# TongtongSong/OpenEAT

Measured on AMD Instinct MI355X. Metric: audio-frames/sec/GPU (train) + RTF (attention-rescoring decode), 12L Conformer, higher is better.
Workload: dtype f32 (storage, accumulate, softmax, norms, losses, optimizer all fp32; every matrix product is the fp32 product to within one fp32 rounding, computed as six exact bf16 x bf16 MFMA products of three-piece operand splits h+m+l = x, dropped terms < 2^-24 |a||b| - tests hold it to the exact-fp32 mode's t; 1 GPU; configs[1]: 12L Conformer d=256 (12+3+3, h=4, ff=1024, K=15, V=3246), B=32/GPU x 10 s 16 kHz wav (T=998 frames), L=30, CTC+attention joint loss, fbank+fwd+bwd+clip+Adam, dropout 0.1; global_batch=32, parallelism=dp1, hip_graph=True

## Files before the change

### openeat_amd/csrc/gemm_tn.hip

```cpp
#include <stdlib.h>
#include "gemm_common.h"
#include "../../include/openeat_hip.h"

typedef __bf16 bf16x8 __attribute__((ext_vector_type(8)));
typedef __bf16 bf16x4 __attribute__((ext_vector_type(4)));
typedef short s16x4 __attribute__((ext_vector_type(4)));

#define TN_KROWS 32
#define TN_COLS 128
#define TN_PITCH (TN_COLS + 16)
#define TN_PLANE (TN_KROWS * TN_PITCH)
#define TN_THREADS 512

#ifdef OE_GEMM_STAMPS
static __device__ unsigned long long* tn_stamp_buf = nullptr;
extern "C" int oe_debug_set_tn_stamp_buffer(void* p) { return (int)hipMemcpyToSymbol(HIP_SYMBOL(tn_stamp_buf), &p, sizeof(p)); }
#define TN_NOW(var)                                                                          \
    do {                                                                                     \
        __builtin_amdgcn_sched_barrier(0);                                                   \
        asm volatile("s_memtime %0\n\ts_waitcnt lgkmcnt(0)" : "=s"(var) :: "memory");        \
        __builtin_amdgcn_sched_barrier(0);                                                   \
    } while (0)
#define TN_ACC(slot) do { unsigned long long t1_; TN_NOW(t1_); tn_acc[slot] += t1_ - tn_t; tn_t = t1_; } while (0)
#else
#define TN_NOW(var) do { } while (0)
#define TN_ACC(slot) do { } while (0)
#endif

template <int TERMS> struct TFrag { bf16x8 p[oe_npl<TERMS>::N]; };

template <int TERMS>
__device__ __forceinline__ void tn_frag(const __bf16* img, int col32, int s, int lane, TFrag<TERMS>& f) {
    const int i = lane & 15, grp = lane >> 4;
    const __bf16* p = img + (16 * s + 4 * (grp >> 1) + (i >> 2)) * TN_PITCH + col32 + 16 * (grp & 1) + 4 * (i & 3);
    typedef __attribute__((address_space(3))) s16x4 lds_s16x4;
#pragma unroll
    for (int n = 0; n < oe_npl<TERMS>::N; ++n) {
        union { s16x4 h[2]; bf16x8 v; } u;
        u.h[0] = __builtin_amdgcn_ds_read_tr16_b64_v4i16((lds_s16x4*)(p + n * TN_PLANE));
        u.h[1] = __builtin_amdgcn_ds_read_tr16_b64_v4i16((lds_s16x4*)(p + n * TN_PLANE + 8 * TN_PITCH));
        f.p[n] = u.v;
    }
}

template <int TERMS>
__device__ __forceinline__ f32x16 tn_mma(const TFrag<TERMS>& a, const TFrag<TERMS>& b, f32x16 c) {
    return oe_mma_terms<TERMS>(a, b, c);
}

struct TnRegs { float4 v[2]; };
__device__ __forceinline__ void tn_load(TnRegs& t, const float* base, long ld, int k0, int k_last) {
#pragma unroll
    for (int i = 0; i < 2; ++i) {
        const int k = min(k0 + (int)(threadIdx.x >> 5) + 16 * i, k_last);
        t.v[i] = *reinterpret_cast<const float4*>(base + (long)k * ld);
    }
}
template <int TERMS>
__device__ __forceinline__ void tn_store(const TnRegs& t, __bf16* img, int k0, int k_end) {
#pragma unroll
    for (int i = 0; i < 2; ++i) {
        const int row = (int)(threadIdx.x >> 5) + 16 * i;
        const bool live = k0 + row < k_end;
        const float x[4] = {live ? t.v[i].x : 0.f, live ? t.v[i].y : 0.f, live ? t.v[i].z : 0.f, live ? t.v[i].w : 0.f};
        constexpr int NPL = oe_npl<TERMS>::N;
        bf16x4 pl[NPL];
#pragma unroll
        for (int e = 0; e < 4; ++e) {
            __bf16 q[NPL];
            oe_split_bf16<NPL>(x[e], q);
#pragma unroll
            for (int n = 0; n < NPL; ++n) pl[n][e] = q[n];
        }
        __bf16* d = img + row * TN_PITCH + 4 * (threadIdx.x & 31);
#pragma unroll
        for (int n = 0; n < NPL; ++n) *reinterpret_cast<bf16x4*>(d + n * TN_PLANE) = pl[n];
    }
}

template <int TERMS>
__device__ __forceinline__ void tn_block(const float* __restrict__ Ap, long lda, const float* __restrict__ Bp, long ldb,
                                         float* __restrict__ C, long ldc, int M, int N, int Mr, int Nr, int K, int k_chunk,
                                         int tile_x, int tile_y, int tile_z, const EpiParams& ep) {
    constexpr int NPL = oe_npl<TERMS>::N;
    constexpr int OP_ELEMS = NPL * TN_PLANE;
    constexpr int BUF_ELEMS = 2 * OP_ELEMS;
    constexpr int XCH_BYTES = 4 * 2 * 32 * 64 * 4;
    constexpr int IMG_ELEMS = (2 * BUF_ELEMS * 2 >= XCH_BYTES) ? 2 * BUF_ELEMS : XCH_BYTES / 2;
    __shared__ __attribute__((aligned(16))) __bf16 img[IMG_ELEMS];
    __shared__ float csum_s[TN_COLS];

    const int lane = threadIdx.x & 63;
    const int wave = __builtin_amdgcn_readfirstlane(threadIdx.x >> 6);
    const int grp = wave >> 2, wm = (wave >> 1) & 1, wn = wave & 1;
    const long m0 = (long)tile_y * TN_COLS, n0 = (long)tile_x * TN_COLS;
    const int k_begin = tile_z * k_chunk;
    const int k_end = min(K, k_begin + k_chunk);
    const int nchunks = (k_end - k_begin + TN_KROWS - 1) / TN_KROWS;

    const int c4 = 4 * (threadIdx.x & 31);
    const float* a_src = Ap + min(m0 + c4, (long)Mr - 4);
    const float* b_src = Bp + min(n0 + c4, (long)Nr - 4);
    const bool do_csum = ep.a_colsum != nullptr && tile_x == 0;
    float cs[4] = {0.f, 0.f, 0.f, 0.f};

    f32x16 acc[2][2];
#pragma unroll
    for (int i = 0; i < 2; ++i)
#pragma unroll
        for (int j = 0; j < 2; ++j)
#pragma unroll
            for (int r = 0; r < 16; ++r) acc[i][j][r] = 0.f;

#ifdef OE_GEMM_STAMPS
    unsigned long long tn_acc[8] = {0, 0, 0, 0, 0, 0, 0, 0}, tn_t, tn_t0;
    TN_NOW(tn_t);
    tn_t0 = tn_t;
#endif
    TnRegs ra, rb;
    if (nchunks > 0) {
        tn_load(ra, a_src, lda, k_begin, k_end - 1);
        tn_load(rb, b_src, ldb, k_begin, k_end - 1);
        if (do_csum) {
#pragma unroll
            for (int i = 0; i < 2; ++i)
                if (k_begin + (int)(threadIdx.x >> 5) + 16 * i < k_end) { cs[0] += ra.v[i].x; cs[1] += ra.v[i].y; cs[2] += ra.v[i].z; cs[3] += ra.v[i].w; }
        }
        tn_store<TERMS>(ra, img, k_begin, k_end);
        tn_store<TERMS>(rb, img + OP_ELEMS, k_begin, k_end);
    }
    __syncthreads();
    TN_ACC(0);
    for (int c = 0; c < nchunks; ++c) {
        const int kn = k_begin + (c + 1) * TN_KROWS;
        const bool more = c + 1 < nchunks;
        if (more) {
            tn_load(ra, a_src, lda, kn, k_end - 1);
            tn_load(rb, b_src, ldb, kn, k_end - 1);
        }
        TN_ACC(1);
        const __bf16* ia = img + (c & 1) * BUF_ELEMS;
        const __bf16* ib = ia + OP_ELEMS;
        TFrag<TERMS> fa[2], fb[2];
        tn_frag<TERMS>(ia, wm * 64, grp, lane, fa[0]);
        tn_frag<TERMS>(ia, wm * 64 + 32, grp, lane, fa[1]);
        tn_frag<TERMS>(ib, wn * 64, grp, lane, fb[0]);
        tn_frag<TERMS>(ib, wn * 64 + 32, grp, lane, fb[1]);
#pragma unroll
        for (int i = 0; i < 2; ++i)
#pragma unroll
            for (int j = 0; j < 2; ++j) acc[i][j] = tn_mma<TERMS>(fa[i], fb[j], acc[i][j]);
        TN_ACC(2);
#ifdef OE_GEMM_STAMPS
        asm volatile("s_waitcnt vmcnt(0)" ::: "memory");
        TN_ACC(3);
#endif
        if (more) {
            if (do_csum) {
#pragma unroll
                for (int i = 0; i < 2; ++i)
                    if (kn + (int)(threadIdx.x >> 5) + 16 * i < k_end) { cs[0] += ra.v[i].x; cs[1] += ra.v[i].y; cs[2] += ra.v[i].z; cs[3] += ra.v[i].w; }
            }
            __bf16* nx = img + ((c + 1) & 1) * BUF_ELEMS;
            tn_store<TERMS>(ra, nx, kn, k_end);
            tn_store<TERMS>(rb, nx + OP_ELEMS, kn, k_end);
        }
        TN_ACC(4);
        __syncthreads();
        TN_ACC(5);
    }

    float alpha = ep.alpha;
    if (ep.alpha_dev) alpha *= *ep.alpha_dev;

    if (do_csum) {
        if (threadIdx.x < TN_COLS) csum_s[threadIdx.x] = 0.f;
        __syncthreads();
#pragma unroll
        for (int e = 0; e < 4; ++e) {
            const float v = cs[e] + __shfl_xor(cs[e], 32, 64);
            if (lane < 32) atomicAdd(&csum_s[4 * lane + e], v);
        }
        __syncthreads();
        if (threadIdx.x < TN_COLS && m0 + threadIdx.x < M) atomicAdd(ep.a_colsum + m0 + threadIdx.x, csum_s[threadIdx.x] * alpha);
    }

    float* xch = reinterpret_cast<float*>(img);
    const int q = wave & 3;
    {
        float* mine = xch + ((q * 2 + grp) * 32) * 64 + lane;
#pragma unroll
        for (int j = 0; j < 2; ++j)
#pragma unroll
            for (int r = 0; r < 16; ++r) mine[(j * 16 + r) * 64] = grp == 0 ? acc[1][j][r] : acc[0][j][r];
    }
    __syncthreads();
    f32x16 fin[2];
    {
        const float* theirs = xch + ((q * 2 + (1 - grp)) * 32) * 64 + lane;
#pragma unroll
        for (int j = 0; j < 2; ++j)
#pragma unroll
            for (int r = 0; r < 16; ++r) fin[j][r] = (grp == 0 ? acc[0][j][r] : acc[1][j][r]) + theirs[(j * 16 + r) * 64];
    }
    const int lrow = lane & 31, lk = lane >> 5;
    const bool interior = (m0 + TN_COLS <= M) && (n0 + TN_COLS <= N);
#pragma unroll
    for (int j = 0; j < 2; ++j) {
        const long col = n0 + wn * 64 + j * 32 + lrow;
        const long row0 = m0 + wm * 64 + grp * 32 + 4 * lk;
        float* base = C + row0 * ldc + col;
#pragma unroll
        for (int r = 0; r < 16; ++r) {
            const int dr = (r & 3) + 8 * (r >> 2);
            if (!interior && !(row0 + dr < M && col < N)) continue;
            const float v = fin[j][r] * alpha;
            if (ep.atomic) atomicAdd(base + dr * ldc, v);
            else if (ep.accumulate) base[dr * ldc] += v;
            else base[dr * ldc] = v;
        }
    }
#ifdef OE_GEMM_STAMPS
    TN_ACC(6);
    if (tn_stamp_buf && threadIdx.x == 0 && blockIdx.x < 2048) {
        for (int i = 0; i < 7; ++i) tn_stamp_buf[blockIdx.x * 8 + i] = tn_acc[i];
        tn_stamp_buf[blockIdx.x * 8 + 7] = tn_t - tn_t0;
    }
#endif
}

__device__ __forceinline__ int tn_swizzle(int id, int nblk) {
    const int q = nblk >> 3, r = nblk & 7, xcd = id & 7, j = id >> 3;
    return (xcd < r ? xcd * (q + 1) : r * (q + 1) + (xcd - r) * q) + j;
}

template <int TERMS>
__global__ __launch_bounds__(TN_THREADS) void gemm_tn_planes_kernel(const float* __restrict__ Ap, long lda, const float* __restrict__ Bp, long ldb,
                                                                   float* __restrict__ C, long ldc, int M, int N, int Mr, int Nr, int K, int k_chunk,
                                                                   int gx, int gy, EpiParams ep) {
    const int swz = tn_swizzle(blockIdx.x, gridDim.x);
    tn_block<TERMS>(Ap, lda, Bp, ldb, C, ldc, M, N, Mr, Nr, K, k_chunk, swz % gx, (swz / gx) % gy, swz / (gx * gy), ep);
}

template <int TERMS>
__global__ __launch_bounds__(TN_THREADS) void gemm_tn_grouped_kernel(const oe_tn_problem* __restrict__ tab, int n_problems) {
    const int swz = tn_swizzle(blockIdx.x, gridDim.x);
    int p = 0;
    while (p + 1 < n_problems && tab[p + 1].block_start <= swz) ++p;
    const oe_tn_problem pr = tab[p];
    const int local = swz - pr.block_start;
    EpiParams ep{};
    ep.alpha = pr.alpha; ep.alpha_dev = pr.alpha_dev; ep.beta = 1.f; ep.atomic = 1; ep.a_colsum = pr.a_colsum;
    tn_block<TERMS>(pr.a, pr.lda, pr.b, pr.ldb, pr.c, pr.ldc, pr.m, pr.n, (pr.m + 3) / 4 * 4, (pr.n + 3) / 4 * 4, pr.k, pr.k_chunk,
                    local % pr.gx, (local / pr.gx) % pr.gy, local / (pr.gx * pr.gy), ep);
}

extern "C" int oe_gemm_tn_grouped_plan(oe_tn_problem* problems, int n, int target_blocks) {
    OE_REQUIRE(problems && n > 0 && target_blocks > 0, "oe_gemm_tn_grouped_plan: bad arguments");
    long tiles = 0;
    for (int i = 0; i < n; ++i) {
        oe_tn_problem& p = problems[i];
        OE_REQUIRE(p.a && p.b && p.c && p.m >= 4 && p.n >= 4 && p.k >= 1, "oe_gemm_tn_grouped_plan: problem %d: bad shape / null pointer", i);
        OE_REQUIRE((((uintptr_t)p.a | (uintptr_t)p.b) & 15) == 0 && p.lda % 4 == 0 && p.ldb % 4 == 0 && p.lda >= (p.m + 3) / 4 * 4 &&
                       p.ldb >= (p.n + 3) / 4 * 4 && p.ldc >= p.n,
                   "oe_gemm_tn_grouped_plan: problem %d: operands not 16-byte aligned / leading dimensions too short", i);
        p.gx = oe_cdiv(p.n, TN_COLS);
        p.gy = oe_cdiv(p.m, TN_COLS);
        tiles += (long)p.gx * p.gy;
    }
    const int split = (int)min(16L, max(1L, (target_blocks + tiles / 2) / tiles));
    int blocks = 0;
    for (int i = 0; i < n; ++i) {
        oe_tn_problem& p = problems[i];
        int nz = min(split, max(1, p.k / 128));
        p.k_chunk = oe_cdiv(oe_cdiv(p.k, nz), TN_KROWS) * TN_KROWS;
        p.nz = oe_cdiv(p.k, p.k_chunk);
        p.block_start = blocks;
        blocks += p.gx * p.gy * p.nz;
    }
    return blocks;
}

extern "C" int oe_gemm_tn_grouped(const oe_tn_problem* problems_dev, int n, int total_blocks, int precision, void* stream) {
    OE_REQUIRE(problems_dev && n > 0 && total_blocks > 0, "oe_gemm_tn_grouped: bad arguments");
    OE_REQUIRE(precision == 1 || precision == 3 || precision == 6, "oe_gemm_tn_grouped: precision must be 1 (bf16), 3 (bf16x3) or 6 (bf16x6)");
    if (precision == 6)
        hipLaunchKernelGGL((gemm_tn_grouped_kernel<6>), dim3(total_blocks), dim3(TN_THREADS), 0, (hipStream_t)stream, problems_dev, n);
    else if (precision == 3)
        hipLaunchKernelGGL((gemm_tn_grouped_kernel<3>), dim3(total_blocks), dim3(TN_THREADS), 0, (hipStream_t)stream, problems_dev, n);
    else
        hipLaunchKernelGGL((gemm_tn_grouped_kernel<1>), dim3(total_blocks), dim3(TN_THREADS), 0, (hipStream_t)stream, problems_dev, n);
    OE_LAUNCH_CHECK("oe_gemm_tn_grouped");
    return 0;
}

int oe_gemm_tn_planes_try(const OperandDesc& A, const OperandDesc& B, float* C, long ldc, int M, int N, int K, int sk, const EpiParams& ep,
                          int terms, hipStream_t st) {
    static const int mode = getenv("OE_GEMM_TN_PLANES") ? atoi(getenv("OE_GEMM_TN_PLANES")) : 1;
    if (!mode) return 1;
    const int Mr = (M + 3) / 4 * 4, Nr = (N + 3) / 4 * 4;
    if (!A.vec_ok || !B.vec_ok || A.ld < Mr || B.ld < Nr || M < 4 || N < 4 || K < 1) return 1;
    if (ep.bias || ep.act || ep.preact_out || ep.actgrad_in || ep.residual || ep.rowmask || ep.drop_p > 0.f || ep.beta != 1.f || ep.scatter) return 1;
    if (sk > 1 && !ep.atomic) return 1;
    const int gx = oe_cdiv(N, TN_COLS), gy = oe_cdiv(M, TN_COLS);
    if (mode == 1 && (gx * gy < 12 || K < 2048)) return 1;
    int nz = 1;
    static const int blocks_target = getenv("OE_TN_BLOCKS") ? atoi(getenv("OE_TN_BLOCKS")) : 256;
    if (ep.atomic) {
        nz = max(1, blocks_target / (gx * gy));
        nz = min(nz, max(1, K / 128));
    }
    int kc = oe_cdiv(oe_cdiv(K, nz), TN_KROWS) * TN_KROWS;
    nz = oe_cdiv(K, kc);
    if (terms == 6)
        hipLaunchKernelGGL((gemm_tn_planes_kernel<6>), dim3(gx * gy * nz), dim3(TN_THREADS), 0, st, A.p, A.ld, B.p, B.ld, C, ldc, M, N, Mr, Nr, K, kc, gx, gy, ep);
    else if (terms == 3)
        hipLaunchKernelGGL((gemm_tn_planes_kernel<3>), dim3(gx * gy * nz), dim3(TN_THREADS), 0, st, A.p, A.ld, B.p, B.ld, C, ldc, M, N, Mr, Nr, K, kc, gx, gy, ep);
    else
        hipLaunchKernelGGL((gemm_tn_planes_kernel<1>), dim3(gx * gy * nz), dim3(TN_THREADS), 0, st, A.p, A.ld, B.p, B.ld, C, ldc, M, N, Mr, Nr, K, kc, gx, gy, ep);
    OE_LAUNCH_CHECK("oe_gemm (bf16 mfma, k-major planes)");
    return 0;
}
```

### openeat_amd/ops.py

```python
from __future__ import annotations

import itertools
import os
import math
import weakref
from typing import Optional

import torch

from . import hip
from . import arena as _arena
from . import planes as _planes

ACT_NONE, ACT_RELU, ACT_SWISH, ACT_TANH, ACT_HARDTANH, ACT_SELU, ACT_GELU = 0, 1, 2, 3, 4, 5, 6
ACT_IDS = {"relu": ACT_RELU, "swish": ACT_SWISH, "tanh": ACT_TANH, "hardtanh": ACT_HARDTANH, "selu": ACT_SELU, "gelu": ACT_GELU,
           "none": ACT_NONE}
GEMM_FUSED_ACTS = (ACT_NONE, ACT_RELU, ACT_SWISH)


_seed_counter = itertools.count(0x5EED0001)
_seed_dev: Optional[torch.Tensor] = None


def next_seed() -> int:
# ... 215 lines not shown
            return None
        hip.call("oe_rowgemm6_pack_table", _ROW.dev, _ROW.n, max(_row_pieces(k) for k in _ROW.entries))
        _pack_done(_ROW)
        for e in _ROW.entries.values():
            o = e["owner"]()
            e["gen"], e["ver"] = gen, (None if o is None else o._version)
    else:
        _pack_wait(_ROW)
    return ent["buf"]


def _rowgemm_try(x, w, transposed, bias, out, epi, ln_pending=None, lnf_pending=None, ln_epi=None):
    try:
        return _rowgemm_try_impl(x, w, transposed, bias, out, epi, ln_pending, lnf_pending, ln_epi)
    finally:
        if ln_pending is not None:
            ln_pending.resolve()
        if lnf_pending is not None:
            lnf_pending.resolve()


def _rowgemm_try_impl(x, w, transposed, bias, out, epi, ln_pending, lnf_pending=None, ln_epi=None):
    if not ROWGEMM or hip.GEMM_PRECISION != 6 or not x.is_cuda:
        return None
    k = x.shape[1]
    n = w.shape[1] if transposed else w.shape[0]
    if (w.shape[0] if transposed else w.shape[1]) != k:
        return None
    form = hip.lib().oe_rowgemm6_form(x.shape[0], k, n)
    if form == 0 or (form == 1 and x.shape[0] < ROWGEMM_MIN_ROWS) or (form == 2 and not ROWTILE):
        return None
    ok = _ROW_EPI_OK if form == 1 else _ROWTILE_EPI_OK
    for key, v in epi.items():
        unset = v is None or (not isinstance(v, torch.Tensor) and (v is False or v == 0 or (key == "beta" and v == 1.0)))
        if not unset and key not in ok:
            return None
    act = epi.get("act", 0) or 0
    pre_out, aux_in, ld_aux = epi.get("preact_out"), epi.get("actgrad_in"), epi.get("ld_aux", 0) or 0
    if act not in (0, ACT_RELU, ACT_SWISH) or (pre_out is not None and aux_in is not None):
        return None
    for t in (pre_out, aux_in):
        if t is not None and (t.dtype != torch.float32 or t.data_ptr() % 8 or ld_aux % 2):
            return None
    if x.stride(1) != 1 or x.stride(0) % 4 or x.data_ptr() % 16 or w.stride(1) != 1 or w.stride(0) % 4 or w.data_ptr() % 16:
        return None
    res = epi.get("residual")
    if res is not None and (res.stride(-1) != 1 or res.data_ptr() % 16 or epi.get("ldr", 0) % 4):
        return None
    if bias is not None and bias.data_ptr() % 16:
        return None
    wp = _row_packed(w, transposed)
    if wp is None:
        return None
    M = x.shape[0]
    if out is None:
        out = _new(M, n, like=x)
    elif out.stride(1) != 1 or out.stride(0) % 4 or out.data_ptr() % 16:
        return None
    global ROWGEMM_LAUNCHES
    ROWGEMM_LAUNCHES += 1
    ln = lnf = None
    if ln_pending is not None and not ln_pending.done:
        sd = epi.get("seed_dev")
        if (form == 1 and k == 256 and x.is_contiguous() and x.data_ptr() == ln_pending.g.data_ptr() and M == ln_pending.rows and
                (sd is None or _seed_dev is None or sd.data_ptr() == _seed_dev.data_ptr()) and (epi.get("drop_p", 0.0) or 0.0) == 0.0):
            ln = ln_pending.prologue()
        else:
            ln_pending.resolve()
    if lnf_pending is not None and not lnf_pending.done:
        q = lnf_pending
        if form == 1 and k == 256 and ln is None and x.is_contiguous() and x.data_ptr() == q.y.data_ptr() and M == q.rows and q.gamma2 is None:
            lnf = q.prologue()
        else:
            q.resolve()
    lne = None
    if (ln_epi is not None and form == 1 and k == 256 and n == 256 and lnf is None and bias is None and not epi and
            M == ln_epi["dx"].shape[0] and ln_epi["dx"].is_contiguous() and ln_epi["x"].is_contiguous()):
        lne = ln_epi
    hip.rowgemm6(x, wp, out, M, k, n, bias=bias, drop_p=epi.get("drop_p", 0.0) or 0.0, seed=epi.get("seed", 0) or 0,
                 seed_dev=(_seed_dev if ln is not None else epi.get("seed_dev")),
                 rowmask=epi.get("rowmask"), residual=res, ldr=epi.get("ldr", 0) or 0, beta=epi.get("beta", 1.0),
                 act=act, preact_out=pre_out, actgrad_in=aux_in, ld_aux=ld_aux, ln=ln, lnf=lnf, lne=lne)
    if lne is not None:
        ln_epi["done"] = True
    if ln is not None:
        ln_pending.fused()
    if lnf is not None:
        lnf_pending.fused()
    return out


def gemm_nt(x, w, bias=None, out=None, out_planes=False, **epi):
    M, K = x.shape
    N = w.shape[0]
    lnf = _PENDING_LNF.take(x)
    if not (out_planes and _planes.split_activations()):
        y = _rowgemm_try(x, w, False, bias, out, epi, lnf_pending=lnf)
        if y is not None:
            return y
    elif lnf is not None:
        lnf.resolve()
    if out is None:
        out = _new(M, N, like=x)
    ap, bp = _operand_planes(x, w)
    cp = _planes.new_output(out) if (out_planes and _planes.split_activations() and out.numel() >= _planes.MIN_SPLIT_ELEMS) else None
    hip.gemm(x, w, out, M, N, K, lda=x.stride(0), ldb=w.stride(0), ldc=out.stride(0), bias=bias, a_planes=ap, b_planes=bp, c_planes=cp, **epi)
    return out


def gemm_nn(dy, w, out=None, out_planes=False, ln_epi=None, **epi):
    M, N = dy.shape
    K = w.shape[1]
    pend = _PENDING_LN.take(dy)
    if not (out_planes and (_planes.available() if out_planes == "always" else _planes.split_activations())):
        y = _rowgemm_try(dy, w, True, None, out, epi, ln_pending=pend, ln_epi=ln_epi)
        if y is not None:
            return y
    elif pend is not None:
        pend.resolve()
    if out is None:
        out = _new(M, K, like=dy)
    ap, bp = _operand_planes(dy, w)
    want = _planes.available() if out_planes == "always" else (out_planes and _planes.split_activations())
    cp = _planes.new_output(out) if (want and out.numel() >= _planes.MIN_SPLIT_ELEMS) else None
    hip.gemm(dy, w, out, M, K, N, lda=dy.stride(0), ldb=w.stride(0), ldc=out.stride(0), b_kmajor=True, a_planes=ap, b_planes=bp, c_planes=cp, **epi)
    return out


def gemm_nn_deep(dy, w, alpha_dev=None):
    M, N = dy.shape
    K = w.shape[1]
    tiles = -(-M // 64) * -(-K // 64)
    sk = 1
    if hip.GEMM_PRECISION != 0 and N >= 2048 and K <= 512:
        want = -(-1984 // tiles)
        sk = 8 if want >= 8 else 4 if want >= 3 else 2
    if sk == 1:
        return gemm_nn(dy, w, alpha_dev=alpha_dev)
    out = _new(M, K, like=dy, zero=True)
    hip.gemm(dy, w, out, M, K, N, lda=dy.stride(0), ldb=w.stride(0), ldc=out.stride(0), b_kmajor=True, split_k=sk,
             atomic_out=True, alpha_dev=alpha_dev)
    return out


def wgrad_planes(dy, x, always=False):
    if not (_planes.available() if always else _planes.active()):
        return None, None
    make = always or _planes.split_activations()
    ap = _planes.of(dy, make=make)
    bp = _planes.of(x, make=make) if ap is not None else None
    return (ap, bp) if bp is not None else (None, None)


def gemm_tn(dy, x, out=None, alpha=1.0, alpha_dev=None, bias_out=None, planes=None):
    M, N = dy.shape
    K = x.shape[1]
    if out is None:
        out = _new(N, K, like=dy, zero=True)
    fused = bias_out is not None and hip.GEMM_PRECISION != 0
    ap, bp = planes if planes is not None else wgrad_planes(dy, x)
    hip.gemm(dy, x, out, N, K, M, lda=dy.stride(0), ldb=x.stride(0), ldc=out.stride(0), a_kmajor=True, b_kmajor=True,
             split_k=_split_k(N, K, M), atomic_out=True, alpha=alpha, alpha_dev=alpha_dev,
             a_colsum=bias_out if fused else None, a_planes=ap, b_planes=bp)
    if bias_out is not None and not fused:
        colsum(dy, alpha, alpha_dev, N, out=bias_out)
    return out


def colsum(x, alpha=1.0, alpha_dev=None, n=None, out=None):
    M = x.shape[0]
    n = x.shape[1] if n is None else n
    acc = out is not None
    if out is None:
        out = _new(n, like=x)
    hip.call("oe_colsum_f32", x, x.stride(0), M, n, alpha, alpha_dev, out, int(acc))
    return out


ASYNC_WGRAD = False
_side_stream = None


def side_stream():
    global _side_stream
    if _side_stream is None:
        _side_stream = torch.cuda.Stream()
    return _side_stream


STAMPS = None


def stamp(tag: str):
    if STAMPS is None:
        return
    slot = len(STAMPS["tags"])
    if slot >= STAMPS["buf"].numel():
        return
    STAMPS["tags"].append(tag)
    hip.call("oe_stamp", STAMPS["buf"], slot)


def stamp_grad(x: torch.Tensor, tag: str) -> None:
    if STAMPS is not None and x.requires_grad:
        x.register_hook(lambda g, tag=tag: stamp(tag))


CUTS = None


def cut(x: torch.Tensor, name: str) -> torch.Tensor:
    if CUTS is None or not x.requires_grad:
        return x
    leaf = x.detach().requires_grad_(True)
    CUTS.append((name, x, leaf))
    return leaf


def forked_streams():
    return [s for s in (_side_stream, _decoder_stream, _ctc_stream) if s is not None] + list(_extra_streams)


_extra_streams = []


def join_side_stream():
    flush_wgrads()
    if _side_stream is not None:
        torch.cuda.current_stream().wait_stream(_side_stream)
    if _decoder_stream is not None:
        torch.cuda.current_stream().wait_stream(_decoder_stream)
    if _ctc_stream is not None:
        torch.cuda.current_stream().wait_stream(_ctc_stream)


PARALLEL_DECODERS = False
_decoder_stream = None


_ctc_stream = None


def ctc_stream():
    global _ctc_stream
    if _ctc_stream is None:
        _ctc_stream = torch.cuda.Stream()
    return _ctc_stream


def decoder_stream():
    global _decoder_stream
    if _decoder_stream is None:
        _decoder_stream = torch.cuda.Stream()
    return _decoder_stream


class _Side:

    def __init__(self, *tensors):
        self.tensors = [t for t in tensors if isinstance(t, torch.Tensor)]

    def __enter__(self):
        side = side_stream()
        side.wait_stream(torch.cuda.current_stream())
        self.cm = torch.cuda.stream(side)
        self.cm.__enter__()

    def __exit__(self, *exc):
        self.cm.__exit__(*exc)
        for t in self.tensors:
            t.record_stream(_side_stream)
        return False


class _Inline:
    def __enter__(self):
        return None

    def __exit__(self, *exc):
        return False


def _wgrad_ctx(to_arena: bool, *tensors):
    return _Side(*tensors) if (ASYNC_WGRAD and to_arena) else _Inline()


WGRAD_DEFER = 0
_deferred = []


def _run_wgrad(to_arena: bool, tensors, fn, desc=None):
    if WGRAD_DEFER > 0 and to_arena:
        _deferred.append((fn, [t for t in tensors if isinstance(t, torch.Tensor)], torch.cuda.current_stream(), desc))
        if len(_deferred) >= WGRAD_DEFER:
            flush_wgrads()
        return
    with _wgrad_ctx(to_arena, *tensors):
        fn()


WGRAD_GROUPED = os.environ.get("OE_WGRAD_GROUPED", "1") == "1"
WGRAD_GROUP_MAX_TILES = int(os.environ.get("OE_WGRAD_GROUP_MAX_TILES", "12"))
WGRAD_GROUP_BLOCKS = int(os.environ.get("OE_WGRAD_GROUP_BLOCKS", "512"))
_TN_TABLES = []


def _group_wgrads(descs):
    if hip.GEMM_PRECISION == 0:
        return set()
    idx = []
    for i, d in enumerate(descs):
        if d is None:
            continue
        dy, x, out = d["dy"], d["x"], d["out"]
        tiles = -(-dy.shape[1] // 128) * -(-x.shape[1] // 128)
        ok = (dy.dim() == 2 and x.dim() == 2 and out.dim() == 2 and dy.stride(1) == 1 and x.stride(1) == 1 and out.stride(1) == 1 and
              dy.shape[0] == x.shape[0] and dy.shape[0] >= 128 and tiles <= WGRAD_GROUP_MAX_TILES and dy.shape[1] >= 4 and x.shape[1] >= 4 and
              dy.stride(0) % 4 == 0 and x.stride(0) % 4 == 0 and dy.data_ptr() % 16 == 0 and x.data_ptr() % 16 == 0 and
              dy.stride(0) >= -(-dy.shape[1] // 4) * 4 and x.stride(0) >= -(-x.shape[1] // 4) * 4)
        if ok:
            idx.append(i)
    if len(idx) < 2:
        return set()
    plan = hip.tn_grouped_plan([descs[i] for i in idx], WGRAD_GROUP_BLOCKS)
    if plan is None:
        return set()
    host, total = plan
    table = torch.empty(len(host), dtype=torch.uint8, device=descs[idx[0]]["dy"].device)
    if LN_TABLE is not None and not LN_TABLE.eager:
        LN_TABLE.uploads.append((table, host))
    else:
        pinned = torch.frombuffer(bytearray(host), dtype=torch.uint8).pin_memory()
        table.copy_(pinned, non_blocking=True)
        _TN_TABLES.append((table, pinned))
        del _TN_TABLES[:-64]
    hip.tn_grouped_launch(table, len(idx), total,
                          flops=sum(2.0 * descs[i]["dy"].shape[0] * descs[i]["dy"].shape[1] * descs[i]["x"].shape[1] for i in idx))
    return set(idx)


def drop_deferred():
    global _deferred
    _deferred = []


WGRAD_FLUSH_INLINE = False


def flush_wgrads():
    global _deferred
    if not _deferred:
        return
    if WGRAD_FLUSH_INLINE:
        grouped = _group_wgrads([d for _, _, _, d in _deferred]) if WGRAD_GROUPED else set()
        for i, (fn, _, _, _) in enumerate(_deferred):
            if i not in grouped:
                fn()
        _deferred = []
        return
    side = side_stream()
    origins = []
    for _, _, st, _ in _deferred:
        if all(st != o for o in origins):
            origins.append(st)
    for st in origins:
        side.wait_stream(st)
    with torch.cuda.stream(side):
        grouped = _group_wgrads([d for _, _, _, d in _deferred]) if WGRAD_GROUPED else set()
        for i, (fn, _, _, _) in enumerate(_deferred):
            if i not in grouped:
                fn()
    for _, ts, _, _ in _deferred:
        for t in ts:
            t.record_stream(side)
    _deferred = []


def wgrad(param, dy, x, alpha=1.0, alpha_dev=None):
    tgt = _arena.grad_target(param)
    if tgt is None:
        return gemm_tn(dy, x, alpha=alpha, alpha_dev=alpha_dev).view(param.shape)
    out = tgt.view(dy.shape[1], x.shape[1])
    pl = wgrad_planes(dy, x)
    _run_wgrad(True, (dy, x, alpha_dev) + _pl_tensors(pl), lambda: gemm_tn(dy, x, out=out, alpha=alpha, alpha_dev=alpha_dev, planes=pl),
               desc=dict(dy=dy, x=x, out=out, alpha=alpha, alpha_dev=alpha_dev, bias_out=None))
    return None


def _pl_tensors(pl):
    return tuple(q.t for q in pl if q is not None) if pl is not None else ()


def _sink_swapped(param, src, A, Bd, Cd):
    tgt = _arena.grad_target(param)
    if tgt is None:
        out = torch.empty_like(param)
        hip.call("oe_swap_last2", src, A, Bd, Cd, out, 0)
        return out
    hip.call("oe_swap_last2", src, A, Bd, Cd, tgt, 1)
    return None


def wgrad_bias(w, b, dy, x, alpha=1.0, alpha_dev=None):
    if b is None:
        return wgrad(w, dy, x, alpha, alpha_dev), None
    N, K = dy.shape[1], x.shape[1]
    tw, tb = _arena.grad_target(w), _arena.grad_target(b)
    ow = tw.view(N, K) if tw is not None else _new(N, K, like=dy, zero=True)
    ob = tb if tb is not None else _new(N, like=dy, zero=True)
    pl = wgrad_planes(dy, x)
    _run_wgrad(tw is not None and tb is not None, (dy, x, alpha_dev) + _pl_tensors(pl),
               lambda: gemm_tn(dy, x, out=ow, alpha=alpha, alpha_dev=alpha_dev, bias_out=ob, planes=pl),
               desc=dict(dy=dy, x=x, out=ow, alpha=alpha, alpha_dev=alpha_dev, bias_out=ob))
    return (None if tw is not None else ow.view(w.shape)), (None if tb is not None else ob)


def bgrad(param, dy, alpha=1.0, alpha_dev=None, n=None):
    if param is None:
        return None
    tgt = _arena.grad_target(param)
    if tgt is None:
        return colsum(dy, alpha, alpha_dev, n)
    colsum(dy, alpha, alpha_dev, n, out=tgt)
    return None


def grad_sink(param):
    tgt = _arena.grad_target(param)
    if tgt is None:
        z = torch.zeros_like(param)
        return z, z
    return tgt.view(param.shape), None


def _fused_rows(parts, cat_dim0=True):
    a = _arena.active()
    if a is not None and a.enabled and a.adjacent(*parts):
        rows = sum(p.shape[0] for p in parts)
        return torch.as_strided(parts[0], (rows,) + tuple(parts[0].shape[1:]), parts[0].stride()), True
    return torch.cat(list(parts), 0), False


def dropout_scale(x, alpha=1.0, p=0.0, seed=0, rowmask=None, cols=None):
    out = torch.empty_like(x)
    cols = x.shape[-1] if cols is None else cols
    hip.call("oe_dropout_scale", x, x.numel(), cols, alpha, p, seed, _seed_dev, rowmask, out)
    return out


def _ln_ws(like, rows, d):
    return _new(hip.lib().oe_layernorm_bwd_workspace_floats(rows, d), like=like)


def _ln_fwd(x, gamma, beta, eps, rows, d, rowmask, act, y, stats, planes_out=True):
    pl = _planes.new_output(y.view(rows, d)) if (planes_out and _planes.active() and rows * d >= _planes.MIN_SPLIT_ELEMS) else None
    if pl is None:
        hip.call("oe_layernorm_fwd", x, gamma, beta, eps, rows, d, rowmask, act, y, stats)
    else:
        hip.call("oe_layernorm_fwd_pl", x, gamma, beta, eps, rows, d, rowmask, act, y, stats, pl.t, pl.stride)


LN_TABLE_CAPACITY = 512


class _LnTable:
    __slots__ = ("dev", "eager", "entries", "keep", "max_rows", "max_d", "launched", "uploads")

    def __init__(self, dev, eager):
        self.dev, self.eager, self.entries, self.keep, self.uploads = dev, eager, [], [], []
        self.max_rows, self.max_d, self.launched = 1, 4, 0

    def add(self, ws, rows, d, dg, db):
        self.entries.append((ws.data_ptr(), rows, d, dg.data_ptr(), db.data_ptr()))
        self.keep.append(ws)
        self.max_rows, self.max_d = max(self.max_rows, rows), max(self.max_d, d)


LN_TABLE = None
LN_EAGER_TABLE = os.environ.get("OE_LN_EAGER_TABLE", "1") == "1"
_LN_EAGER_DEV = {}
_LN_EAGER_PINNED = []


def ln_table_begin(device, eager=False):
    global LN_TABLE
    if eager:
        dev = _LN_EAGER_DEV.get(device)
        if dev is None:
            dev = _LN_EAGER_DEV[device] = torch.zeros(LN_TABLE_CAPACITY, 5, dtype=torch.int64, device=device)
    else:
        dev = torch.zeros(LN_TABLE_CAPACITY, 5, dtype=torch.int64, device=device)
    LN_TABLE = _LnTable(dev, eager)
    return LN_TABLE


def ln_table_flush():
    t = LN_TABLE
    if t is None or len(t.entries) == t.launched:
        return
    first, n = t.launched, len(t.entries) - t.launched
    assert len(t.entries) <= LN_TABLE_CAPACITY, "LN_TABLE_CAPACITY exceeded"
    if t.eager:
        host = torch.tensor(t.entries[first:], dtype=torch.int64).pin_memory()
        t.dev[first:first + n].copy_(host, non_blocking=True)
        _LN_EAGER_PINNED.append(host)
        del _LN_EAGER_PINNED[:-8]
        cur = torch.cuda.current_stream()
        for ws in t.keep:
            ws.record_stream(cur)
    hip.call("oe_layernorm_param_reduce_table", t.dev[first:], n, t.max_rows, t.max_d)
    t.launched = len(t.entries)
    t.keep = []


def ln_table_end():
    global LN_TABLE
    t, LN_TABLE = LN_TABLE, None
    if t is not None and t.entries:
        t.dev[: len(t.entries)].copy_(torch.tensor(t.entries, dtype=torch.int64))
    if t is not None:
        for table, host in t.uploads:
            table.copy_(torch.frombuffer(bytearray(host), dtype=torch.uint8))
    return t


def _ln_param_reduce(ws, rows, d, dg, db, to_arena):
    if LN_TABLE is not None and to_arena:
        LN_TABLE.add(ws, rows, d, dg, db)
    else:
        hip.call("oe_layernorm_param_reduce", ws, rows, d, dg, db)


FUSE_OUT_DROP = os.environ.get("OE_FUSE_OUT_DROP", "1") == "1"
_PREDROP = {}


def predrop_clear():
    resolve_pending_ln()
    resolve_pending_lnf()
    _PREDROP.clear()
    _planes.clear()


def _tag_out_drop(out, out_scale, p_out, s_out, rowmask=None, ln_fuse=False):
    if FUSE_OUT_DROP and (p_out > 0 or out_scale != 1.0 or rowmask is not None):
        out._oe_outdrop = (float(out_scale), float(p_out), int(s_out), rowmask)
        if ln_fuse:
            out._oe_lnfuse = True
    return out


LN_BWD_FUSE = os.environ.get("OE_LN_BWD_FUSE", "1") == "1"
LN_BWD_FUSED_LAUNCHES = 0
LN_EPI_FUSE = os.environ.get("OE_LN_EPI_FUSE", "1") == "1"
LN_EPI_FUSED_LAUNCHES = 0
_PENDING_LN = _ParkRegistry("g")


def resolve_pending_ln():
    return _PENDING_LN.sweep()


def _ln_rows_fusable(rows, d):
    return hip.GEMM_PRECISION == 6 and d == 256 and rows >= ROWGEMM_MIN_ROWS and not _planes.active()


def _ln_fuse_ok(rows, d, w):
    return LN_BWD_FUSE and ROWGEMM and FUSE_OUT_DROP and _ln_rows_fusable(rows, d) and w.shape[0] == 256 and w.shape[1] == 256


class _LnBwdPark:
    __slots__ = ("dy", "x", "gamma", "beta", "stats", "add", "dx", "g", "ws", "spec", "rows", "d", "dg", "db", "rowmask",
                 "gamma2", "stats2", "ws2", "dg2", "db2", "table", "done")

    def __init__(self, dy, x, gamma, beta, stats, add, dx, g, ws, spec, rows, d, dg, db, rowmask=None,
                 gamma2=None, stats2=None, ws2=None, dg2=None, db2=None):
        self.dy, self.x, self.gamma, self.beta, self.stats, self.add, self.dx, self.g = dy, x, gamma, beta, stats, add, dx, g
        self.ws, self.spec, self.rows, self.d, self.dg, self.db, self.rowmask = ws, spec, rows, d, dg, db, rowmask
        self.gamma2, self.stats2, self.ws2, self.dg2, self.db2 = gamma2, stats2, ws2, dg2, db2
        self.table, self.done = LN_TABLE is not None, False
        if self.table:
            for args in self._partials():
                LN_TABLE.add(*args)

    def _partials(self):
        one = (self.ws, self.rows, self.d, self.dg, self.db)
        return (one,) if self.gamma2 is None else (one, (self.ws2, self.rows, self.d, self.dg2, self.db2))

    def _launched(self):
        self.done = True
        if not self.table:
            for args in self._partials():
                hip.call("oe_layernorm_param_reduce", *args)

    def resolve(self):
        if self.done:
            return
        alpha, p, seed, gmask = self.spec
        if self.gamma2 is not None:
            hip.call("oe_layernorm_pair_bwd_dx_drop", self.dy, self.x, self.gamma, self.beta, self.stats, self.gamma2, self.stats2,
                     self.rows, self.d, self.add, self.dx, self.g, alpha, p, seed, _seed_dev, gmask, self.ws, self.ws2)
        else:
            hip.call("oe_layernorm_bwd_dx_drop", self.dy, self.x, self.gamma, self.beta, 0, self.stats, self.rows, self.d,
                     self.rowmask, self.add, self.dx, self.g, alpha, p, seed, _seed_dev, gmask, self.ws)
        self._launched()

    def prologue(self):
        alpha, p, seed, gmask = self.spec
        return dict(dy=self.dy, x=self.x, stats=self.stats, gamma=self.gamma, add=self.add, dx=self.dx, g=self.g, ws=self.ws,
                    alpha=alpha, p=p, seed=seed, rowmask=gmask, ln_rowmask=self.rowmask, beta=self.beta if self.gamma2 is not None else None,
                    gamma2=self.gamma2, stats2=self.stats2, ws2=self.ws2)

    def fused(self):
        global LN_BWD_FUSED_LAUNCHES
        LN_BWD_FUSED_LAUNCHES += 1
        self._launched()


def _out_drop_grad(dy2, out_scale, p_out, s_out, rowmask=None):
    hit = _PREDROP.pop(dy2.data_ptr(), None)
    if hit is not None:
        g, spec, dx, version = hit
        same_mask = (spec[3] is None and rowmask is None) or (spec[3] is not None and rowmask is not None and
                                                               spec[3].data_ptr() == rowmask.data_ptr())
        if (dx._version == version and dx.numel() == dy2.numel() and spec[:3] == (float(out_scale), float(p_out), int(s_out)) and
                same_mask and g.numel() == dy2.numel()):
            return g.view(dy2.shape)
        pend = _PENDING_LN.take(g)
        if pend is not None:
            pend.resolve()
    return dropout_scale(dy2, out_scale, p_out, s_out, rowmask)


def _ln_bwd(dy, x, gamma, beta, act, stats, rows, d, rowmask, add, dx, dg, db, to_arena, prev_drop=None, fuse=False):
    ws = _ln_ws(x, rows, d)
    if (fuse and to_arena and prev_drop is not None and LN_BWD_FUSE and FUSE_OUT_DROP and act == ACT_NONE and _ln_rows_fusable(rows, d) and
            dy.is_contiguous() and x.is_contiguous() and (add is None or add.is_contiguous())):
        g = torch.empty_like(dx)
        _PENDING_LN.park(_LnBwdPark(dy, x, gamma, beta, stats, add, dx, g, ws, prev_drop, rows, d, dg, db, rowmask=rowmask))
        _PREDROP[dx.data_ptr()] = (g, prev_drop, dx, dx._version)
        return
# ... 1436 lines not shown
```

Baseline: 1.962 million audio-frames/s.

## Restructure TN wgrad GEMM main loop for multi-stage loads and add wgrad pairing

Rewrites the TN (weight-gradient) GEMM K-loop around a compile-time stage count D. The loop prefetches D chunks into registers, waits with explicit vmcnt limits, and interleaves the LDS split-stores with MFMAs through sched_group_barrier hints. It also folds the column-sum into the store, switches to a vectorised split helper, and adds an optional path in ops.py that groups larger same-shape wgrads into shared grouped launches. With the defaults (stages=2, pair=1) the main change is the scheduling and interleave restructure, which trades compiler freedom and register pressure for better overlap of global loads with compute.

Result: no change. 1.972 million audio-frames/s (median of 6 runs) (+0.5%).

```diff
diff --git a/openeat_amd/csrc/gemm_tn.hip b/openeat_amd/csrc/gemm_tn.hip
--- a/openeat_amd/csrc/gemm_tn.hip
+++ b/openeat_amd/csrc/gemm_tn.hip
@@ -11,6 +11,12 @@
 #define TN_PITCH (TN_COLS + 16)
 #define TN_PLANE (TN_KROWS * TN_PITCH)
 #define TN_THREADS 512
+#ifndef TN_STAGES
+#define TN_STAGES 2
+#endif
+#ifndef TN_INTERLEAVE
+#define TN_INTERLEAVE 1
+#endif
 
 #ifdef OE_GEMM_STAMPS
 static __device__ unsigned long long* tn_stamp_buf = nullptr;
@@ -22,9 +28,11 @@
         __builtin_amdgcn_sched_barrier(0);                                                   \
     } while (0)
 #define TN_ACC(slot) do { unsigned long long t1_; TN_NOW(t1_); tn_acc[slot] += t1_ - tn_t; tn_t = t1_; } while (0)
+#define TN_WAIT(n) asm volatile("s_waitcnt vmcnt(%0)" ::"n"(n) : "memory")
 #else
 #define TN_NOW(var) do { } while (0)
 #define TN_ACC(slot) do { } while (0)
+#define TN_WAIT(n) do { } while (0)
 #endif
 
 template <int TERMS> struct TFrag { bf16x8 p[oe_npl<TERMS>::N]; };
@@ -53,32 +61,39 @@
 #pragma unroll
     for (int i = 0; i < 2; ++i) {
         const int k = min(k0 + (int)(threadIdx.x >> 5) + 16 * i, k_last);
-        t.v[i] = *reinterpret_cast<const float4*>(base + (long)k * ld);
-    }
-}
-template <int TERMS>
-__device__ __forceinline__ void tn_store(const TnRegs& t, __bf16* img, int k0, int k_end) {
+        typedef float f32x4 __attribute__((ext_vector_type(4)));
+        typedef const __attribute__((address_space(1))) f32x4 gf32x4;
+        const f32x4 v = *(gf32x4*)(base + (long)k * ld);
+        t.v[i] = make_float4(v[0], v[1], v[2], v[3]);
+    }
+}
+template <int TERMS>
+__device__ __forceinline__ void tn_store(const TnRegs& t, __bf16* img, int k0, int k_end, float* cs = nullptr) {
 #pragma unroll
     for (int i = 0; i < 2; ++i) {
         const int row = (int)(threadIdx.x >> 5) + 16 * i;
         const bool live = k0 + row < k_end;
         const float x[4] = {live ? t.v[i].x : 0.f, live ? t.v[i].y : 0.f, live ? t.v[i].z : 0.f, live ? t.v[i].w : 0.f};
+        if (cs) {
+#pragma unroll
+            for (int e = 0; e < 4; ++e) cs[e] += x[e];
+        }
         constexpr int NPL = oe_npl<TERMS>::N;
-        bf16x4 pl[NPL];
-#pragma unroll
-        for (int e = 0; e < 4; ++e) {
-            __bf16 q[NPL];
-            oe_split_bf16<NPL>(x[e], q);
-#pragma unroll
-            for (int n = 0; n < NPL; ++n) pl[n][e] = q[n];
-        }
+        oe_bf16x4v pl[NPL];
+        oe_split4<NPL>(x, pl);
         __bf16* d = img + row * TN_PITCH + 4 * (threadIdx.x & 31);
 #pragma unroll
-        for (int n = 0; n < NPL; ++n) *reinterpret_cast<bf16x4*>(d + n * TN_PLANE) = pl[n];
-    }
-}
-
-template <int TERMS>
+        for (int n = 0; n < NPL; ++n) *reinterpret_cast<oe_bf16x4v*>(d + n * TN_PLANE) = pl[n];
+    }
+}
+
+__device__ __forceinline__ void tn_csum(const TnRegs& t, float (&cs)[4], int k0, int k_end) {
+#pragma unroll
+    for (int i = 0; i < 2; ++i)
+        if (k0 + (int)(threadIdx.x >> 5) + 16 * i < k_end) { cs[0] += t.v[i].x; cs[1] += t.v[i].y; cs[2] += t.v[i].z; cs[3] += t.v[i].w; }
+}
+
+template <int TERMS, int D>
 __device__ __forceinline__ void tn_block(const float* __restrict__ Ap, long lda, const float* __restrict__ Bp, long ldb,
                                          float* __restrict__ C, long ldc, int M, int N, int Mr, int Nr, int K, int k_chunk,
                                          int tile_x, int tile_y, int tile_z, const EpiParams& ep) {
@@ -117,28 +132,20 @@
     TN_NOW(tn_t);
     tn_t0 = tn_t;
 #endif
-    TnRegs ra, rb;
-    if (nchunks > 0) {
-        tn_load(ra, a_src, lda, k_begin, k_end - 1);
-        tn_load(rb, b_src, ldb, k_begin, k_end - 1);
-        if (do_csum) {
-#pragma unroll
-            for (int i = 0; i < 2; ++i)
-                if (k_begin + (int)(threadIdx.x >> 5) + 16 * i < k_end) { cs[0] += ra.v[i].x; cs[1] += ra.v[i].y; cs[2] += ra.v[i].z; cs[3] += ra.v[i].w; }
-        }
-        tn_store<TERMS>(ra, img, k_begin, k_end);
-        tn_store<TERMS>(rb, img + OP_ELEMS, k_begin, k_end);
-    }
+    TnRegs ra[D], rb[D];
+    const int k_last = k_end - 1;
+    static_for<0, D>([&](auto s_c) {
+        constexpr int S = decltype(s_c)::value;
+        tn_load(ra[S], a_src, lda, k_begin + S * TN_KROWS, k_last);
+        tn_load(rb[S], b_src, ldb, k_begin + S * TN_KROWS, k_last);
+        __builtin_amdgcn_sched_barrier(0);
+    });
+    if (do_csum) tn_csum(ra[0], cs, k_begin, k_end);
+    tn_store<TERMS>(ra[0], img, k_begin, k_end);
+    tn_store<TERMS>(rb[0], img + OP_ELEMS, k_begin, k_end);
     __syncthreads();
     TN_ACC(0);
-    for (int c = 0; c < nchunks; ++c) {
-        const int kn = k_begin + (c + 1) * TN_KROWS;
-        const bool more = c + 1 < nchunks;
-        if (more) {
-            tn_load(ra, a_src, lda, kn, k_end - 1);
-            tn_load(rb, b_src, ldb, kn, k_end - 1);
-        }
-        TN_ACC(1);
+    auto compute = [&](int c) {
         const __bf16* ia = img + (c & 1) * BUF_ELEMS;
         const __bf16* ib = ia + OP_ELEMS;
         TFrag<TERMS> fa[2], fb[2];
@@ -151,24 +158,54 @@
 #pragma unroll
             for (int j = 0; j < 2; ++j) acc[i][j] = tn_mma<TERMS>(fa[i], fb[j], acc[i][j]);
         TN_ACC(2);
-#ifdef OE_GEMM_STAMPS
-        asm volatile("s_waitcnt vmcnt(0)" ::: "memory");
-        TN_ACC(3);
-#endif
-        if (more) {
-            if (do_csum) {
-#pragma unroll
-                for (int i = 0; i < 2; ++i)
-                    if (kn + (int)(threadIdx.x >> 5) + 16 * i < k_end) { cs[0] += ra.v[i].x; cs[1] += ra.v[i].y; cs[2] += ra.v[i].z; cs[3] += ra.v[i].w; }
+    };
+    int c = 0;
+    for (; c + D < nchunks; c += D) {
+        static_for<0, D>([&](auto s_c) {
+            constexpr int S = decltype(s_c)::value, SN = (S + 1) % D;
+            const int cc = c + S, kn = k_begin + (cc + 1) * TN_KROWS;
+            tn_load(ra[S], a_src, lda, k_begin + (cc + D) * TN_KROWS, k_last);
+            tn_load(rb[S], b_src, ldb, k_begin + (cc + D) * TN_KROWS, k_last);
+            __builtin_amdgcn_sched_barrier(0);
+            TN_ACC(1);
+            compute(cc);
+            TN_WAIT(4 * (D - 1));
+            TN_ACC(3);
+            __bf16* nx = img + ((cc + 1) & 1) * BUF_ELEMS;
+            tn_store<TERMS>(ra[SN], nx, kn, k_end, cs);
+            tn_store<TERMS>(rb[SN], nx + OP_ELEMS, kn, k_end);
+#if TN_INTERLEAVE
+#pragma unroll
+            for (int g = 0; g < 4 * TERMS; ++g) {
+                __builtin_amdgcn_sched_group_barrier(0x008, 1, 0);
+                __builtin_amdgcn_sched_group_barrier(0x002, TERMS == 6 ? 5 : TERMS == 3 ? 6 : 8, 0);
             }
-            __bf16* nx = img + ((c + 1) & 1) * BUF_ELEMS;
-            tn_store<TERMS>(ra, nx, kn, k_end);
-            tn_store<TERMS>(rb, nx + OP_ELEMS, kn, k_end);
+#endif
+            TN_ACC(4);
+            __syncthreads();
+            TN_ACC(5);
+        });
+    }
+    static_for<0, D>([&](auto s_c) {
+        constexpr int S = decltype(s_c)::value, SN = (S + 1) % D;
+        const int cc = c + S, kn = k_begin + (cc + 1) * TN_KROWS;
+        if (cc < nchunks) {
+            compute(cc);
+            if constexpr (S + 1 < D) {
+                if (cc + 1 < nchunks) {
+                    TN_WAIT(4 * (D - 2 - S));
+                    TN_ACC(3);
+                    if (do_csum) tn_csum(ra[SN], cs, kn, k_end);
+                    __bf16* nx = img + ((cc + 1) & 1) * BUF_ELEMS;
+                    tn_store<TERMS>(ra[SN], nx, kn, k_end);
+                    tn_store<TERMS>(rb[SN], nx + OP_ELEMS, kn, k_end);
+                    TN_ACC(4);
+                }
+            }
+            __syncthreads();
+            TN_ACC(5);
         }
-        TN_ACC(4);
-        __syncthreads();
-        TN_ACC(5);
-    }
+    });
 
     float alpha = ep.alpha;
     if (ep.alpha_dev) alpha *= *ep.alpha_dev;
@@ -239,7 +276,7 @@
                                                                    float* __restrict__ C, long ldc, int M, int N, int Mr, int Nr, int K, int k_chunk,
                                                                    int gx, int gy, EpiParams ep) {
     const int swz = tn_swizzle(blockIdx.x, gridDim.x);
-    tn_block<TERMS>(Ap, lda, Bp, ldb, C, ldc, M, N, Mr, Nr, K, k_chunk, swz % gx, (swz / gx) % gy, swz / (gx * gy), ep);
+    tn_block<TERMS, TN_STAGES>(Ap, lda, Bp, ldb, C, ldc, M, N, Mr, Nr, K, k_chunk, swz % gx, (swz / gx) % gy, swz / (gx * gy), ep);
 }
 
 template <int TERMS>
@@ -251,7 +288,7 @@
     const int local = swz - pr.block_start;
     EpiParams ep{};
     ep.alpha = pr.alpha; ep.alpha_dev = pr.alpha_dev; ep.beta = 1.f; ep.atomic = 1; ep.a_colsum = pr.a_colsum;
-    tn_block<TERMS>(pr.a, pr.lda, pr.b, pr.ldb, pr.c, pr.ldc, pr.m, pr.n, (pr.m + 3) / 4 * 4, (pr.n + 3) / 4 * 4, pr.k, pr.k_chunk,
+    tn_block<TERMS, TN_STAGES>(pr.a, pr.lda, pr.b, pr.ldb, pr.c, pr.ldc, pr.m, pr.n, (pr.m + 3) / 4 * 4, (pr.n + 3) / 4 * 4, pr.k, pr.k_chunk,
                     local % pr.gx, (local / pr.gx) % pr.gy, local / (pr.gx * pr.gy), ep);
 }
 
diff --git a/openeat_amd/ops.py b/openeat_amd/ops.py
--- a/openeat_amd/ops.py
+++ b/openeat_amd/ops.py
@@ -541,29 +541,47 @@
 WGRAD_GROUPED = os.environ.get("OE_WGRAD_GROUPED", "1") == "1"
 WGRAD_GROUP_MAX_TILES = int(os.environ.get("OE_WGRAD_GROUP_MAX_TILES", "12"))
 WGRAD_GROUP_BLOCKS = int(os.environ.get("OE_WGRAD_GROUP_BLOCKS", "512"))
+WGRAD_PAIR = int(os.environ.get("OE_WGRAD_PAIR", "1"))
+assert WGRAD_PAIR in (1, 2, 4), "OE_WGRAD_PAIR must be 1, 2 or 4"
+WGRAD_PAIR_BLOCKS = 256
 _TN_TABLES = []
+_TN_TABLES_KEPT = 256
 
 
 def _group_wgrads(descs):
     if hip.GEMM_PRECISION == 0:
         return set()
-    idx = []
+    idx, big = [], {}
     for i, d in enumerate(descs):
         if d is None:
             continue
         dy, x, out = d["dy"], d["x"], d["out"]
         tiles = -(-dy.shape[1] // 128) * -(-x.shape[1] // 128)
         ok = (dy.dim() == 2 and x.dim() == 2 and out.dim() == 2 and dy.stride(1) == 1 and x.stride(1) == 1 and out.stride(1) == 1 and
-              dy.shape[0] == x.shape[0] and dy.shape[0] >= 128 and tiles <= WGRAD_GROUP_MAX_TILES and dy.shape[1] >= 4 and x.shape[1] >= 4 and
+              dy.shape[0] == x.shape[0] and dy.shape[0] >= 128 and dy.shape[1] >= 4 and x.shape[1] >= 4 and
               dy.stride(0) % 4 == 0 and x.stride(0) % 4 == 0 and dy.data_ptr() % 16 == 0 and x.data_ptr() % 16 == 0 and
               dy.stride(0) >= -(-dy.shape[1] // 4) * 4 and x.stride(0) >= -(-x.shape[1] // 4) * 4)
-        if ok:
+        if not ok:
+            continue
+        if tiles <= WGRAD_GROUP_MAX_TILES:
             idx.append(i)
-    if len(idx) < 2:
-        return set()
-    plan = hip.tn_grouped_plan([descs[i] for i in idx], WGRAD_GROUP_BLOCKS)
+        elif WGRAD_PAIR > 1 and tiles * WGRAD_PAIR <= WGRAD_PAIR_BLOCKS // 4:
+            big.setdefault((dy.shape[0], tiles), []).append(i)
+    covered = set()
+    if len(idx) >= 2 and _launch_wgrad_group(descs, idx, WGRAD_GROUP_BLOCKS):
+        covered.update(idx)
+    for members in big.values():
+        for j in range(0, len(members) - WGRAD_PAIR + 1, WGRAD_PAIR):
+            grp = members[j:j + WGRAD_PAIR]
+            if _launch_wgrad_group(descs, grp, WGRAD_PAIR_BLOCKS):
+                covered.update(grp)
+    return covered
+
+
+def _launch_wgrad_group(descs, idx, target_blocks):
+    plan = hip.tn_grouped_plan([descs[i] for i in idx], target_blocks)
     if plan is None:
-        return set()
+        return False
     host, total = plan
     table = torch.empty(len(host), dtype=torch.uint8, device=descs[idx[0]]["dy"].device)
     if LN_TABLE is not None and not LN_TABLE.eager:
@@ -572,10 +590,10 @@
         pinned = torch.frombuffer(bytearray(host), dtype=torch.uint8).pin_memory()
         table.copy_(pinned, non_blocking=True)
         _TN_TABLES.append((table, pinned))
-        del _TN_TABLES[:-64]
+        del _TN_TABLES[:-_TN_TABLES_KEPT]
     hip.tn_grouped_launch(table, len(idx), total,
                           flops=sum(2.0 * descs[i]["dy"].shape[0] * descs[i]["dy"].shape[1] * descs[i]["x"].shape[1] for i in idx))
-    return set(idx)
+    return True
 
 
 def drop_deferred():
```
